# cvlab-epfl/gecco

Hardware: AMD Instinct MI355X
Metric: denoiser_fwd_points_per_sec (higher is better)
Workload: dtype f16/fp6/fp8 mixed (the mixed mode with the point MLP of every layer as ONE launch: fp16 main products + fp6 block-scaled second terms for AdaGN(x) and both weights, the 768-wide hidden layer kept in registers as fp16; the other sites as in the mixed mode; fp32 accumulate, residual stream and statist; 1 GPU; C2 unconditional denoiser forward: B=64/GPU, N=2048, d=384, L=6, I=64, H=8, EDMPrecond(LinearLift(SetTransformer)), mixed fp16 / fp6- and fp8-cross-term MFMA, one-launch point MLP, random-init weights; parallelism=single GPU

## Files before the change

gecco_amd/_lib.py:

```python
from __future__ import annotations

import ctypes as C
import os

_HERE = os.path.dirname(os.path.abspath(__file__))
LIB_PATH = os.environ.get("GECCO_HIP_LIB") or os.path.join(_HERE, "libgecco_hip.so")
ABI_VERSION = 14

c_f = C.c_void_p


class GeccoAdaGN(C.Structure):
    _fields_ = [("scale_w", c_f), ("scale_b", c_f), ("bias_w", c_f), ("bias_b", c_f)]


class GeccoMLP(C.Structure):
    _fields_ = [("w0", c_f), ("b0", c_f), ("alpha", c_f), ("w2", c_f), ("b2", c_f)]


class GeccoLayer(C.Structure):
    _fields_ = [("broadcast_norm", GeccoAdaGN), ("inducers", c_f), ("kv_proj_w", c_f), ("pool_out_w", c_f),
                ("norm_1", GeccoAdaGN), ("bmlp", GeccoMLP), ("norm_2", GeccoAdaGN), ("in_proj_w", c_f),
                ("in_proj_b", c_f), ("unpool_out_w", c_f), ("unpool_out_b", c_f), ("mlp_norm", GeccoAdaGN),
                ("mlp", GeccoMLP)]
# ... 64 lines not shown
    "gecco_split_f16_image_bytes": (sz, [i, i]),
    "gecco_linear_image_ok_f16": (i, [i, i, i, i]),
    "gecco_linear_actbwd_ok": (i, [i, i, i, i]),
    "gecco_linear_actbwd_tiles": (sz, [i, i, i]),
    "gecco_linear_actbwd_f32": (i, [vp, vp, vp, vp, i, vp, vp, vp, i, i, i, i, i, vp, vp]),
    "gecco_linear_act_keep_f32": (i, [vp, vp, vp, vp, i, vp, vp, i, i, i, i, i, vp, vp]),
    "gecco_linear_act_keep_pro_f32": (i, [vp, vp, vp, vp, vp, vp, i, vp, vp, i, i, i, i, i, vp, vp]),
    "gecco_linear_f16io": (i, [vp] * 7 + [i, i, i, i, i, i, i, vp, vp]),
    "gecco_linear_pair_f16io": (i, [vp, vp, vp, i, vp, vp, vp, i, vp, i, i, i, vp, vp]),
    "gecco_mlp_fused_f16": (i, [vp, vp, vp, vp, vp, vp, vp, vp, i, vp, i, i, i, i, vp, vp]),
    "gecco_unpool_outproj_f16": (i, [vp, vp, vp, vp, vp, vp, i, i, i, i, vp, vp]),
    "gecco_unpool_outproj_h8": (i, [vp, vp, vp, vp, vp, vp, i, i, i, i, vp, vp]),
    "gecco_mlp_fused_w": (i, [vp, vp, vp, vp, vp, vp, vp, vp, vp, i, vp, i, i, i, i, vp, vp, vp]),
    "gecco_mlp_fused_w_wsplit_bytes": (sz, [i, i]),
    "gecco_unpool_outproj_h8_wsplit_bytes": (sz, [i, i, i]),
    "gecco_unpool_attn_h8img": (i, [vp, vp, vp, i, i, i, i, vp]),
    "gecco_gemm_tn_x3_f32": (i, [vp, vp, vp, i, i, i, i, i, vp]),
    "gecco_gemm_tn_x3_bias_f32": (i, [vp, vp, vp, vp, i, i, i, i, i, vp]),
    "gecco_gemm_tn_x3_pro_f32": (i, [vp, vp, vp, vp, vp, vp, i, i, i, i, i, vp]),
    "gecco_gemm_tn_f16_f32": (i, [vp, vp, vp, vp, vp, vp, i, i, i, i, i, vp]),
    "gecco_gemm_tn_f16_tiles": (i, [i, i]),
    "gecco_gemm_tn_f16_b16_f32": (i, [vp, vp, vp, vp, i, i, i, i, i, vp]),
    "gecco_gemm_tn_f16_a16_f32": (i, [vp, vp, vp, vp, vp, vp, i, i, i, i, i, vp]),
    "gecco_gemm_tn_f16_ex_f32": (i, [vp, i, vp, i, vp, vp, vp, vp, vp, vp, vp, i, i, i, i, i, vp]),
    "gecco_linear_dotstats_a16_f32": (i, [vp] * 6 + [i, i, i, i, vp, vp]),
    "gecco_linear_astat16_actbwd_h16": (i, [vp] * 4 + [i, vp, vp, i, i, i, i, vp, vp]),
    "gecco_linear_dotstats_f32": (i, [vp] * 5 + [i, i, i, i, i, vp, vp]),
    "gecco_h8_image_bytes": (sz, [i, i]),
    "gecco_linear_h8_train_ok": (i, [i, i, i]),
    "gecco_h8_images_f32": (i, [C.POINTER(GeccoSplitJob), i, vp]),
    "gecco_linear_h8_train_f32": (i, [vp] * 5 + [i, vp, vp, vp, i, vp, vp, i, vp, i, i, i, vp, vp]),
    "gecco_astat16_image_bytes": (sz, [i, i]),
    "gecco_linear_astat16_ok": (i, [i, i, i]),
    "gecco_astat16_images_f32": (i, [C.POINTER(GeccoSplitJob), i, vp]),
    "gecco_linear_astat16_f32": (i, [vp] * 5 + [i, vp, vp, vp, i, vp, vp, i, i, i, i, vp, vp]),
    "gecco_linear_astat16_keep": (i, [vp] * 6 + [i, vp, vp, i, i, i, i, vp, vp]),
    "gecco_linear_astat16_keep_y16": (i, [vp] * 6 + [i, vp, vp, vp, i, i, i, i, vp, vp]),
    "gecco_linear_astat16_actbwd": (i, [vp] * 4 + [i, vp, vp, i, i, i, i, vp, vp]),
    "gecco_linear_act_keep_h16": (i, [vp] * 6 + [i, vp, vp, i, i, i, i, vp, vp]),
    "gecco_set_option": (i, [C.c_char_p, i]),
    "gecco_option_index": (i, [C.c_char_p]),
    "gecco_cast_f16": (i, [c_f, C.c_void_p, C.c_size_t, C.c_void_p]),
    "gecco_linear_astat_f16": (i, [vp, vp, vp, vp, vp, i, vp, vp, vp, i, vp, vp, i, i, i, i, i, vp, vp]),
    "gecco_linear_kvq_f16": (i, [vp, vp, vp, vp, vp, i, vp, vp, vp, i, vp, i, i, i, i, i, i, vp, vp]),
    "gecco_linear_kvq_y16_f16": (i, [vp, vp, vp, vp, vp, i, vp, vp, vp, i, vp, vp, i, i, i, i, i, i, vp, vp]),
    "gecco_linear_h8_img_f32": (i, [vp, vp, vp, vp, vp, vp, i, vp, i, i, i, i, i, vp, vp]),
    "gecco_linear_h8_areg_f32": (i, [vp, vp, vp, vp, vp, vp, i, i, i, i, vp, vp]),
    "gecco_affine_cast_f16": (i, [vp, vp, vp, vp, i, i, i, vp]),
    "gecco_pool_attn_f16in": (i, [vp, vp, vp, i, i, i, i, i, i, vp, sz, vp]),
    "gecco_unpool_attn_f16io": (i, [vp, vp, vp, i, i, i, i, i, i, vp]),
    "gecco_lift0_fold_f32": (i, [vp] * 8 + [i, i, i, vp]),
    "gecco_lift0_rows": (i, [vp, vp, vp, vp, i, i, i, i, i, i, i, vp]),
    "gecco_lift0_pool_f32": (i, [vp] * 5 + [i, i, i, i, vp, sz, vp]),
    "gecco_col_stats_f32": (i, [vp, vp, i, i, i, vp]),
    "gecco_stats_row_tiles": (i, [i]),
    "gecco_adagn_coeffs_f32": (i, [vp, i, i, vp, i, C.POINTER(GeccoAdaGN), vp, vp, i, i, i, fl, vp]),
    "gecco_affine_apply_f32": (i, [vp, vp, vp, vp, i, i, i, vp]),
    "gecco_adagn_f32": (i, [vp, vp, i, C.POINTER(GeccoAdaGN), vp, i, i, i, i, fl, vp, sz, vp]),
    "gecco_adagn_workspace_bytes": (sz, [i, i, i]),
    "gecco_pool_attn_f32": (i, [vp, vp, vp, i, i, i, i, i, vp, sz, vp]),
    "gecco_pool_attn_ex_f32": (i, [vp, vp, vp, i, i, i, i, i, i, vp, sz, vp]),
    "gecco_pool_attn_workspace_bytes": (sz, [i, i, i, i, i]),
    "gecco_unpool_attn_f32": (i, [vp, vp, vp, i, i, i, i, i, vp]),
    "gecco_unpool_attn_ex_f32": (i, [vp, vp, vp, i, i, i, i, i, i, vp]),
    "gecco_pool_attn_lse_f32": (i, [vp, sz, vp, i, i, i, i, i, vp]),
    "gecco_pool_attn_bwd_partials": (i, [i, i, i]),
    "gecco_pool_attn_bwd_f32": (i, [vp] * 7 + [i, i, i, i, i, vp]),
    "gecco_unpool_attn_bwd_partials": (i, [i, i, i]),
    "gecco_unpool_attn_bwd_f32": (i, [vp] * 5 + [i, i, i, i, i, vp]),
    "gecco_pool_attn_bwd_ex_f32": (i, [vp] * 7 + [i, i, i, i, i, i, vp]),
    "gecco_unpool_attn_bwd_ex_f32": (i, [vp] * 5 + [i, i, i, i, i, i, vp]),
    "gecco_edm_coeffs_f32": (i, [vp, fl, vp, i, vp]),
    "gecco_lift_f32": (i, [vp, vp, vp, vp, vp, vp, i, i, i, vp]),
    "gecco_lower_edm_f32": (i, [vp] * 9 + [i, i, i, fl, vp]),
    "gecco_set_transformer_fwd_f32": (i, [C.POINTER(GeccoSetTransformer), vp, vp, vp, i, PP, PP, vp, i, i, vp, sz, vp]),
    "gecco_set_transformer_workspace_bytes": (sz, [C.POINTER(GeccoSetTransformer), i, i]),
    "gecco_linear_lift_fwd_f32": (i, [C.POINTER(GeccoLinearLift), vp, vp, vp, vp, PP, PP, i, i, vp, sz, vp]),
    "gecco_linear_lift_workspace_bytes": (sz, [C.POINTER(GeccoLinearLift), i, i]),
    "gecco_lift_g_f32": (i, [vp, vp, vp, vp, vp, vp, i, i, i, i, vp]),
    "gecco_lower_edm_g_f32": (i, [vp] * 7 + [i, i, i, i, i, fl, vp]),
    "gecco_linear_lift_g_fwd_f32": (i, [C.POINTER(GeccoLinearLiftG), vp, vp, vp, vp, PP, PP, i, i, vp, sz, vp]),
    "gecco_linear_lift_g_workspace_bytes": (sz, [C.POINTER(GeccoLinearLiftG), i, i]),
    "gecco_nchw_to_nhwc_f32": (i, [vp, vp, i, i, i, i, vp]),
    "gecco_bilinear_taps_f32": (i, [vp, i, i, vp, vp, vp, vp, sz, vp]),
    "gecco_ray_lookup_taps_f32": (i, [vp, vp, vp, vp, vp, vp, vp, vp, vp, vp, i, i, vp]),
    "gecco_ray_lookup_f32": (i, [vp, vp, vp, C.POINTER(GeccoReparam), C.POINTER(GeccoPyramid), vp, vp, i, i, vp]),
    "gecco_lookup_row_tiles": (i, [i]),
    "gecco_ray_lookup_bwd_f32": (i, [vp, vp, vp, C.POINTER(GeccoReparam), C.POINTER(GeccoPyramid), vp, PP, i, i, vp]),
    "gecco_ray_lookup_dgeom_f32": (i, [vp, vp, C.POINTER(GeccoReparam), C.POINTER(GeccoPyramid), vp, vp, vp, i, i, vp]),
    "gecco_ray_lookup_bwd_sorted_workspace_bytes": (C.c_size_t, [C.POINTER(GeccoPyramid), i, i]),
    "gecco_ray_lookup_bwd_sorted_f32": (i, [vp, vp, vp, C.POINTER(GeccoReparam), C.POINTER(GeccoPyramid), vp, PP, i, i, vp,
                                            C.c_size_t, vp]),
    "gecco_ray_network_fwd_f32": (i, [C.POINTER(GeccoRayNetwork), vp, vp, vp, C.POINTER(GeccoPyramid), vp, vp, PP, PP,
                                      i, i, vp, sz, vp]),
    "gecco_ray_network_workspace_bytes": (sz, [C.POINTER(GeccoRayNetwork), C.POINTER(GeccoPyramid), i, i]),
    "gecco_gaussian_reparam": (i, [vp, vp, vp, vp, sz, i, i, i, vp]),
    "gecco_uvl_reparam": (i, [vp, vp, vp, vp, db, vp, i, i, i, i, vp]),
    "gecco_gaussian_act_f32": (i, [vp, vp, vp, sz, i, vp]),
    "gecco_relu_f32": (i, [vp, vp, sz, vp]),
    "gecco_relu_bwd_f32": (i, [vp, vp, vp, sz, vp]),
    "gecco_sampler_add_noise_f64": (i, [vp, vp, sz, vp, vp, i, i, vp, vp, vp, sz, i, vp]),
    "gecco_sampler_add_noise_f32": (i, [vp, vp, sz, vp, vp, i, vp, vp, sz, i, vp]),
    "gecco_sampler_euler_f64": (i, [vp, vp, vp, vp, vp, vp, vp, vp, sz, i, vp]),
    "gecco_sampler_heun_f64": (i, [vp, vp, vp, vp, vp, vp, vp, sz, vp]),
    "gecco_sampler_advance": (i, [vp, i, vp]),
    "gecco_sampler_scale_f64": (i, [vp, db, vp, sz, vp]),
# ... 101 lines not shown
```

gecco_amd/csrc/api_model_ops.hip:

```cpp
#include "api_common.h"

#include <math.h>

using namespace gecco_api;

int gecco_api::make_lookup_args(const GeccoReparam* rp, const GeccoPyramid* pyr, LookupArgs* a) {
    if (!pyr || pyr->n_levels < 1 || pyr->n_levels > 4) return fail(-8, "lookup: 1..4 pyramid levels required");
    a->n_levels = pyr->n_levels;
    a->c_total = 0;
    for (int l = 0; l < 4; ++l) {
        const bool on = l < pyr->n_levels;
        a->C[l] = on ? pyr->C[l] : 0;
        a->H[l] = on ? pyr->H[l] : 1;
        a->W[l] = on ? pyr->W[l] : 1;
        a->feat[l] = on ? pyr->feat[l] : nullptr;
        if (on && !pyr->feat[l]) return fail(-1, "lookup: null pyramid level %d", l);
        a->c_total += a->C[l];
    }
    a->texel_f16 = pyr->texel_f16 ? 1 : 0;
    a->out_f16 = 0;
    a->reparam_kind = rp ? rp->kind : 0;
    a->rp_mean = rp ? rp->mean : nullptr;
    a->rp_std = rp ? rp->std : nullptr;
    a->logit_scale = rp ? rp->logit_scale : 1.1f;
    if (a->reparam_kind && (!a->rp_mean || !a->rp_std)) return fail(-1, "lookup: reparam buffers missing");
    return 0;
}

extern "C" {

int gecco_affine_cast_f16(const float* x, const float* a, const float* o, void* y16, int B, int rows, int C,
                          void* stream) {
    if (C % 8) return fail(-2, "affine_cast_f16: C must be a multiple of 8");
    TRY(affine_cast_f16_launch(x, a, o, y16, B, rows, C, (hipStream_t)stream), "affine_cast_f16");
    return 0;
}

int gecco_pool_attn_f16in(const void* KV16, const float* inducers, float* merged, int B, int N, int C, int H, int I,
                          int head_major, void* ws, size_t ws_bytes, void* stream) {
    if (ws_bytes < gecco_pool_attn_workspace_bytes(B, N, C, H, I)) return fail(-7, "pool_attn: workspace too small");
    Carver c(ws);
    const int ns = pool_attn_nsplit(B, N, H);
    float* po = c.f32((size_t)B * H * ns * 64 * (C / H));
    float* pml = c.f32((size_t)B * H * ns * 64 * 2);
    int rc = pool_attn_launch(static_cast<const float*>(KV16), inducers, po, pml, merged, B, N, C, H, I, ns,
                              (hipStream_t)stream, 2, 1, head_major != 0);
    if (rc == -9) return fail(-2, "pool_attn_f16in: head dim must be 16, 32, 48 or 64");
    TRY(rc, "pool_attn_f16in");
    return 0;
}

int gecco_lift0_fold_f32(const float* kv_w, const float* q_w, const float* q_b, const float* lift_w, const float* lift_b, const float* a1,
                         const float* o1, float* mc, int B, int C, int H, void* stream) {
    if (!kv_w || !q_w || !lift_w || !a1 || !o1 || !mc) return fail(-1, "lift0_fold: null argument");
    if (!lift0_supported(C, H)) return fail(-2, "lift0_fold: feature_dim must be a multiple of 8 and of the head count, at most 1024");
    TRY(lift0_fold_launch(kv_w, q_w, q_b, lift_w, lift_b, a1, o1, mc, 0, 3 * C, B, C, (hipStream_t)stream), "lift0_fold");
    return 0;
}

int gecco_lift0_rows(const float* x, const float* coef, const float* mc, void* out, int col0, int ncols, int head_dim, int out_f16,
                     int B, int N, int C, void* stream) {
    if (!x || !coef || !mc || !out) return fail(-1, "lift0_rows: null argument");
    if (ncols <= 0 || ncols % 8 || col0 < 0 || col0 + ncols > 3 * C) return fail(-2, "lift0_rows: columns must be a multiple of 8 inside 0 .. 3 * feature_dim");
    if (head_dim && (!lift0_head_major_ok(head_dim) || ncols % head_dim)) return fail(-2, "lift0_rows: head dim %d has no head-major form", head_dim);
    const Lift0Seg seg{out, col0, ncols, head_dim};
    TRY(lift0_rows_launch(x, coef, mc, &seg, 1, out_f16 != 0, B, N, C, (hipStream_t)stream), "lift0_rows");
    return 0;
}

int gecco_lift0_pool_f32(const float* x, const float* coef, const float* mc, const float* inducers, float* merged, int B, int N, int C,
                         int H, void* ws, size_t ws_bytes, void* stream) {
    if (!x || !coef || !mc || !inducers || !merged || !ws) return fail(-1, "lift0_pool: null argument");
    if (!lift0_pool_supported(C, H)) return fail(-2, "lift0_pool: feature_dim must be a multiple of 8, at most 1024, the head dim a multiple of 4");
    if (ws_bytes < gecco_pool_attn_workspace_bytes(B, N, C, H, 64)) return fail(-7, "lift0_pool: workspace too small");
    Carver c(ws);
    const int ns = pool_attn_nsplit(B, N, H);
    float* po = c.f32((size_t)B * H * ns * 64 * (C / H));
    float* pml = c.f32((size_t)B * H * ns * 64 * 2);
    TRY(lift0_pool_launch(x, coef, mc, inducers, po, pml, B, N, C, H, ns, (hipStream_t)stream), "lift0_pool");
    TRY(pool_merge_launch(po, pml, merged, B, C, H, ns, (hipStream_t)stream), "lift0_pool merge");
    return 0;
}

int gecco_unpool_attn_f16io(const void* q16, const float* kvh, void* out16, int B, int N, int C, int H, int I,
                            int head_major, void* stream) {
    int rc = unpool_attn_launch(static_cast<const float*>(q16), kvh, static_cast<float*>(out16), B, N, C, H, I,
                                (hipStream_t)stream, 2, 1, head_major != 0);
    if (rc == -9) return fail(-2, "unpool_attn_f16io: head dim must be 16, 32, 48 or 64");
    TRY(rc, "unpool_attn_f16io");
    return 0;
}

int gecco_col_stats_f32(const float* x, float* stats, int B, int rows, int C, void* stream) {
    TRY(col_stats_launch(x, stats, B, rows, C, (hipStream_t)stream), "col_stats");
    return 0;
}

int gecco_adagn_coeffs_f32(const float* stats, int T, int rows, const float* t, int ctx_dim, const GeccoAdaGN* p,
                           float* a, float* o, int B, int C, int G, float eps, void* stream) {
    TRY(adagn_coeffs_launch(stats, T, rows, t, ctx_dim, p ? p->scale_w : nullptr, p ? p->scale_b : nullptr,
                            p ? p->bias_w : nullptr, p ? p->bias_b : nullptr, a, o, B, C, G, eps,
                            (hipStream_t)stream), "adagn_coeffs");
    return 0;
}

int gecco_affine_apply_f32(const float* x, const float* a, const float* o, float* y, int B, int rows, int C,
                           void* stream) {
    TRY(affine_apply_launch(x, a, o, y, B, rows, C, (hipStream_t)stream), "affine_apply");
    return 0;
}

size_t gecco_adagn_workspace_bytes(int B, int rows, int C) {
    Carver c(nullptr);
    c.f32((size_t)B * row_tiles_stats(rows) * 2 * C);
    c.f32((size_t)B * C);
    c.f32((size_t)B * C);
    return (c.off + 255) & ~size_t(255);
}

int gecco_adagn_f32(const float* x, const float* t, int ctx_dim, const GeccoAdaGN* p, float* y, int B, int rows,
                    int C, int G, float eps, void* ws, size_t ws_bytes, void* stream) {
    if (ws_bytes < gecco_adagn_workspace_bytes(B, rows, C)) return fail(-7, "adagn: workspace too small");
    Carver c(ws);
    float* stats = c.f32((size_t)B * row_tiles_stats(rows) * 2 * C);
    float* a = c.f32((size_t)B * C);
    float* o = c.f32((size_t)B * C);
    hipStream_t s = (hipStream_t)stream;
    TRY(col_stats_launch(x, stats, B, rows, C, s), "col_stats");
    TRY(adagn_coeffs_launch(stats, row_tiles_stats(rows), rows, t, ctx_dim, p ? p->scale_w : nullptr,
                            p ? p->scale_b : nullptr, p ? p->bias_w : nullptr, p ? p->bias_b : nullptr, a, o, B, C, G,
                            eps, s), "adagn_coeffs");
    TRY(affine_apply_launch(x, a, o, y, B, rows, C, s), "affine_apply");
    return 0;
}
// ... 525 lines not shown
```

gecco_amd/csrc/lift0.hip:

```cpp
#include "common.h"
#include "kernels.h"

namespace {

constexpr float LOG2E = 1.4426950408889634f;
constexpr int FOLD_MAX_C = 1024;
constexpr int ROWS_THREADS = 192;
constexpr int ROWS_TILE = 256;
constexpr int POOL_WAVES = 16;

typedef unsigned u32x4 __attribute__((ext_vector_type(4)));

__global__ __launch_bounds__(256) void lift0_fold_kernel(const float* __restrict__ kv_w, const float* __restrict__ q_w,
                                                         const float* __restrict__ q_b, const float* __restrict__ lift_w,
                                                         const float* __restrict__ lift_b, const float* __restrict__ a1,
                                                         const float* __restrict__ o1, float4* __restrict__ mc, int row0,
                                                         int row1, int C) {
    __shared__ float4 g[FOLD_MAX_C];
    const int b = blockIdx.y;
    for (int k = threadIdx.x; k < C; k += 256) {
        const float a = a1[(size_t)b * C + k], o = o1[(size_t)b * C + k];
        g[k] = make_float4(a * lift_w[k * 3 + 0], a * lift_w[k * 3 + 1], a * lift_w[k * 3 + 2], fmaf(a, lift_b ? lift_b[k] : 0.f, o));
    }
    __syncthreads();
    const int j = row0 + blockIdx.x * 256 + threadIdx.x;
    if (j >= row1) return;
    const f32x4* wr = reinterpret_cast<const f32x4*>(j < 2 * C ? kv_w + (size_t)j * C : q_w + (size_t)(j - 2 * C) * C);
    float4 acc[4];
#pragma unroll
    for (int e = 0; e < 4; ++e) acc[e] = make_float4(0.f, 0.f, 0.f, 0.f);
#pragma unroll 4
    for (int k4 = 0; k4 < C / 4; ++k4) {
        const f32x4 wv = wr[k4];
#pragma unroll
        for (int e = 0; e < 4; ++e) {
            const float4 gk = g[k4 * 4 + e];
            acc[e].x = fmaf(wv[e], gk.x, acc[e].x); acc[e].y = fmaf(wv[e], gk.y, acc[e].y);
            acc[e].z = fmaf(wv[e], gk.z, acc[e].z); acc[e].w = fmaf(wv[e], gk.w, acc[e].w);
        }
    }
    const float bias = (j >= 2 * C && q_b) ? q_b[j - 2 * C] : 0.f;
    mc[(size_t)b * 3 * C + j] = make_float4(((acc[0].x + acc[1].x) + acc[2].x) + acc[3].x, ((acc[0].y + acc[1].y) + acc[2].y) + acc[3].y,
                                            ((acc[0].z + acc[1].z) + acc[2].z) + acc[3].z, (((acc[0].w + acc[1].w) + acc[2].w) + acc[3].w) + bias);
}

struct RowsSeg {
    void* out;
    int col0, gw, ngroups, hm;
    int ld;
};

template <bool F16>
__global__ __launch_bounds__(ROWS_THREADS) void lift0_rows_kernel(const float* __restrict__ x, const float* __restrict__ coef,
                                                                  const float4* __restrict__ mc, RowsSeg s0, RowsSeg s1, int N,
                                                                  int C) {
    __shared__ float xs[ROWS_TILE * 3];
    const int b = blockIdx.z, n0 = blockIdx.x * ROWS_TILE, rows = min(ROWS_TILE, N - n0);
    const bool first = (int)blockIdx.y < s0.ngroups;
    const RowsSeg& s = first ? s0 : s1;
    const int grp = first ? blockIdx.y : blockIdx.y - s0.ngroups;
    const float cin = coef[4 * b + 2];
    for (int i = threadIdx.x; i < rows * 3; i += ROWS_THREADS) xs[i] = cin * x[((size_t)b * N + n0) * 3 + i];
    const int P = s.gw >> 3, piece = threadIdx.x % P, rstep = ROWS_THREADS / P;
    float4 m[8];
    const float4* mp = mc + (size_t)b * 3 * C + s.col0 + grp * s.gw + piece * 8;
#pragma unroll
    for (int e = 0; e < 8; ++e) m[e] = mp[e];
    __syncthreads();
    const size_t base = s.hm ? ((size_t)(b * s.ngroups + grp) * N + n0) * s.gw + piece * 8
                             : ((size_t)b * N + n0) * s.ld + grp * s.gw + piece * 8;
    const size_t rstride = s.hm ? s.gw : s.ld;
    for (int r = threadIdx.x / P; r < rows; r += rstep) {
        const float p0 = xs[r * 3 + 0], p1 = xs[r * 3 + 1], p2 = xs[r * 3 + 2];
        float v[8];
#pragma unroll
        for (int e = 0; e < 8; ++e) v[e] = fmaf(p2, m[e].z, fmaf(p1, m[e].y, fmaf(p0, m[e].x, m[e].w)));
        if (F16) {
            u32x4 o;
#pragma unroll
            for (int e = 0; e < 4; ++e) {
                typedef _Float16 h2 __attribute__((ext_vector_type(2)));
                const h2 pk = {(_Float16)v[2 * e], (_Float16)v[2 * e + 1]};
                o[e] = __builtin_bit_cast(unsigned, pk);
            }
            *reinterpret_cast<u32x4*>(static_cast<_Float16*>(s.out) + base + r * rstride) = o;
        } else {
            float* dst = static_cast<float*>(s.out) + base + r * rstride;
            *reinterpret_cast<f32x4*>(dst) = f32x4{v[0], v[1], v[2], v[3]};
            *reinterpret_cast<f32x4*>(dst + 4) = f32x4{v[4], v[5], v[6], v[7]};
        }
    }
}

__global__ __launch_bounds__(POOL_WAVES * 64) void lift0_pool_kernel(const float* __restrict__ x, const float* __restrict__ coef,
                                                                     const float4* __restrict__ mc, const float* __restrict__ ind,
                                                                     float* __restrict__ part_o, float* __restrict__ part_ml, int N,
                                                                     int C, int H, int HD, int nsplit) {
    constexpr int NW = POOL_WAVES;
    __shared__ float4 red[NW][64];
    __shared__ float redl[NW][64];
    const int lane = threadIdx.x & 63;
    int wave = __builtin_amdgcn_readfirstlane(threadIdx.x >> 6);
    asm volatile("" : "+s"(wave));
    const int bh = blockIdx.x / nsplit, split = blockIdx.x % nsplit;
    const int b = bh / H, hh = bh % H;
    const int ks = (((N + nsplit - 1) / nsplit) + 31) / 32 * 32;
    const int k_begin = split * ks, k_end = min(N, k_begin + ks);
    const int cnt = max(k_end - k_begin, 0);
    const float cin = coef[4 * b + 2];
    const float4* mk = mc + (size_t)b * 3 * C + hh * HD;
    const float4* mv = mk + C;
    typedef const __attribute__((address_space(4))) float* cfloat_p;
    const cfloat_p xp = (cfloat_p)(x + ((size_t)b * N + k_begin) * 3);

    {
        const float scale = LOG2E * rsqrtf((float)HD);
        const float* qi = ind + ((size_t)hh * 64 + lane) * HD;
        float4 acc = make_float4(0.f, 0.f, 0.f, 0.f);
        for (int d0 = wave * 4; d0 < HD; d0 += NW * 4) {
            const f32x4 q4 = *reinterpret_cast<const f32x4*>(qi + d0);
#pragma unroll
            for (int e = 0; e < 4; ++e) {
                const float4 k4 = mk[d0 + e];
                const float qs = q4[e] * scale;
                acc.x = fmaf(qs, k4.x, acc.x); acc.y = fmaf(qs, k4.y, acc.y); acc.z = fmaf(qs, k4.z, acc.z); acc.w = fmaf(qs, k4.w, acc.w);
            }
        }
        red[wave][lane] = acc;
    }
    __syncthreads();
    float4 u = red[0][lane];
#pragma unroll
    for (int w = 1; w < NW; ++w) { const float4 t = red[w][lane]; u.x += t.x; u.y += t.y; u.z += t.z; u.w += t.w; }
    __syncthreads();
    u.x *= cin; u.y *= cin; u.z *= cin;
    auto score = [&](float p0, float p1, float p2) { return fmaf(u.z, p2, fmaf(u.y, p1, fmaf(u.x, p0, u.w))); };

    float m = -INFINITY, l = 0.f, sx = 0.f, sy = 0.f, sz = 0.f;
    for (int k = wave; k < cnt; k += 4 * NW) {
        float p[4][3], sc[4];
#pragma unroll
        for (int j = 0; j < 4; ++j) {
            const int kk = k + j * NW, kc = min(kk, cnt - 1);
#pragma unroll
            for (int e = 0; e < 3; ++e) p[j][e] = xp[kc * 3 + e];
            sc[j] = kk < cnt ? score(p[j][0], p[j][1], p[j][2]) : -INFINITY;
        }
        const float mn = fmaxf(fmaxf(m, fmaxf(sc[0], sc[1])), fmaxf(sc[2], sc[3]));
        const float a = __builtin_amdgcn_exp2f(m - mn);
        l *= a; sx *= a; sy *= a; sz *= a;
#pragma unroll
        for (int j = 0; j < 4; ++j) {
            const float e = __builtin_amdgcn_exp2f(sc[j] - mn);
            l += e;
            sx = fmaf(e, p[j][0], sx); sy = fmaf(e, p[j][1], sy); sz = fmaf(e, p[j][2], sz);
        }
        m = mn;
    }
    redl[wave][lane] = m;
    red[wave][lane] = make_float4(sx, sy, sz, l);
    __syncthreads();
    float M = redl[0][lane];
#pragma unroll
    for (int w = 1; w < NW; ++w) M = fmaxf(M, redl[w][lane]);
    float4 S = make_float4(0.f, 0.f, 0.f, 0.f);
#pragma unroll
    for (int w = 0; w < NW; ++w) {
        const float mw = redl[w][lane];
        const float f = mw == -INFINITY ? 0.f : exp2f(mw - M);
        const float4 t = red[w][lane];
        S.x = fmaf(f, t.x, S.x); S.y = fmaf(f, t.y, S.y); S.z = fmaf(f, t.z, S.z); S.w = fmaf(f, t.w, S.w);
    }
    S.x *= cin; S.y *= cin; S.z *= cin;
    const size_t pbase = ((size_t)bh * nsplit + split) * 64 + lane;
    for (int d = wave; d < HD; d += NW) {
        const float4 v4 = mv[d];
        part_o[pbase * HD + d] = fmaf(v4.z, S.z, fmaf(v4.y, S.y, fmaf(v4.x, S.x, v4.w * S.w)));
    }
    if (wave == 0) {
        part_ml[pbase * 2 + 0] = M;
        part_ml[pbase * 2 + 1] = S.w;
    }
}

int group_width(int ncols) {
    for (int gw : {64, 48, 32, 16, 8})
        if (ncols % gw == 0) return gw;
    return 0;
}

}

bool lift0_supported(int C, int H) { return C >= 8 && C % 8 == 0 && C <= FOLD_MAX_C && H > 0 && C % H == 0; }
bool lift0_head_major_ok(int hd) { return hd >= 8 && hd % 8 == 0 && ROWS_THREADS % (hd / 8) == 0; }
bool lift0_pool_supported(int C, int H) { return lift0_supported(C, H) && (C / H) % 4 == 0; }

int lift0_fold_launch(const float* kv_w, const float* q_w, const float* q_b, const float* lift_w, const float* lift_b, const float* a1,
                      const float* o1, float* mc, int row0, int row1, int B, int C, hipStream_t st) {
    if (C > FOLD_MAX_C || row0 < 0 || row1 > 3 * C || row0 >= row1 || (row0 < 2 * C && !kv_w) || (row1 > 2 * C && !q_w)) return -3;
    if (B <= 0) return 0;
    hipLaunchKernelGGL(lift0_fold_kernel, dim3((row1 - row0 + 255) / 256, B), dim3(256), 0, st, kv_w, q_w, q_b, lift_w, lift_b, a1, o1,
                       reinterpret_cast<float4*>(mc), row0, row1, C);
    return (int)hipGetLastError();
}

int lift0_rows_launch(const float* x, const float* coef, const float* mc, const Lift0Seg* segs, int nseg, int f16, int B, int N, int C,
                      hipStream_t st) {
    if (nseg < 1 || nseg > 2 || B > 65535) return -3;
    if (B <= 0 || N <= 0) return 0;
    RowsSeg rs[2] = {};
    for (int i = 0; i < nseg; ++i) {
        const Lift0Seg& s = segs[i];
        if (s.ncols <= 0 || s.ncols % 8 || s.col0 < 0 || s.col0 + s.ncols > 3 * C) return -3;
        if (s.hd && (!lift0_head_major_ok(s.hd) || s.ncols % s.hd)) return -3;
        const int gw = s.hd ? s.hd : group_width(s.ncols);
        rs[i] = RowsSeg{s.out, s.col0, gw, s.ncols / gw, s.hd != 0, s.ncols};
    }
    const dim3 grid((N + ROWS_TILE - 1) / ROWS_TILE, rs[0].ngroups + rs[1].ngroups, B);
    if (f16) hipLaunchKernelGGL(lift0_rows_kernel<true>, grid, dim3(ROWS_THREADS), 0, st, x, coef, reinterpret_cast<const float4*>(mc), rs[0], rs[1], N, C);
    else hipLaunchKernelGGL(lift0_rows_kernel<false>, grid, dim3(ROWS_THREADS), 0, st, x, coef, reinterpret_cast<const float4*>(mc), rs[0], rs[1], N, C);
    return (int)hipGetLastError();
}

int lift0_pool_launch(const float* x, const float* coef, const float* mc, const float* inducers, float* part_o, float* part_ml, int B,
                      int N, int C, int H, int nsplit, hipStream_t st) {
    if (!lift0_pool_supported(C, H) || nsplit < 1) return -3;
    if (B <= 0) return 0;
    hipLaunchKernelGGL(lift0_pool_kernel, dim3(B * H * nsplit), dim3(POOL_WAVES * 64), 0, st, x, coef, reinterpret_cast<const float4*>(mc), inducers,
                       part_o, part_ml, N, C, H, C / H, nsplit);
    return (int)hipGetLastError();
}
```

gecco_amd/hip_ops.py:

```python
from __future__ import annotations

import contextlib
import ctypes as C
import itertools
import os
import threading
from typing import Mapping, Sequence

import torch
from torch import Tensor

from . import _lib
from ._lib import GeccoAdaGN, GeccoLayer, GeccoLinearLift, GeccoMLP, GeccoSetTransformer, check

GN_EPS = 1e-5

PRECISIONS = {"fp32": 0, "bf16x3": 1, "fp16": 2, "mixed": 3, "w2": 4}
_default_precision = os.environ.get("GECCO_PRECISION", "fp32")


def set_default_precision(name: str) -> None:
    global _default_precision
    if name not in PRECISIONS:
        raise ValueError(f"precision must be one of {sorted(PRECISIONS)}")
# ... 360 lines not shown
    B, _, N, hd = q16.shape
    Cc = H * hd
    out = torch.empty(B, N // 128, Cc // 64, 24576, device=q16.device, dtype=torch.uint8)
    check(lib.gecco_unpool_attn_h8img(_ptr16(q16), _ptr(kvh), C.c_void_p(out.data_ptr()), B, N, Cc, H, _stream()), "gecco_unpool_attn_h8img")
    return out


def affine_cast_f16(x: Tensor, a: Tensor, o: Tensor, out: Tensor | None = None) -> Tensor:
    lib = _lib.load()
    B, rows, Cc = x.shape
    out = torch.empty(B, rows, Cc, device=x.device, dtype=torch.float16) if out is None else out
    check(lib.gecco_affine_cast_f16(_ptr(x), _ptr(a), _ptr(o), _ptr16(out), B, rows, Cc, _stream()), "gecco_affine_cast_f16")
    return out


def pool_attn_f16in(KV16: Tensor, inducers: Tensor, H: int, head_major: bool = False) -> Tensor:
    lib = _lib.load()
    if head_major:
        B, _, N, hd = KV16.shape
        Cc = H * hd
    else:
        B, N, C2 = KV16.shape
        Cc = C2 // 2
    I = inducers.shape[-2]
    merged = torch.empty(B, I, Cc, device=KV16.device, dtype=torch.float32)
    nb = lib.gecco_pool_attn_workspace_bytes(B, N, Cc, H, I)
    ws = _ws(nb, KV16.device)
    check(lib.gecco_pool_attn_f16in(_ptr16(KV16), _ptr(inducers), _ptr(merged), B, N, Cc, H, I, int(head_major),
                                    C.c_void_p(ws.data_ptr()), nb, _stream()), "gecco_pool_attn_f16in")
    return merged


def lift0_fold(kv_w: Tensor, in_proj_w: Tensor, in_proj_b: Tensor | None, lift_w: Tensor, lift_b: Tensor | None, a1: Tensor, o1: Tensor,
               H: int) -> Tensor:
    lib = _lib.load()
    B, Cc = a1.shape
    mc = torch.empty(B, 3 * Cc, 4, device=a1.device, dtype=torch.float32)
    check(lib.gecco_lift0_fold_f32(_ptr(kv_w), _ptr(in_proj_w), _ptr(in_proj_b), _ptr(lift_w), _ptr(lift_b), _ptr(a1), _ptr(o1), _ptr(mc),
                                   B, Cc, H, _stream()), "gecco_lift0_fold_f32")
    return mc


def lift0_rows(x: Tensor, coef: Tensor, mc: Tensor, col0: int, ncols: int, head_dim: int = 0, f16: bool = True) -> Tensor:
    lib = _lib.load()
    B, N, _ = x.shape
    Cc = mc.shape[1] // 3
    shape = (B, ncols // head_dim, N, head_dim) if head_dim else (B, N, ncols)
    out = torch.empty(*shape, device=x.device, dtype=torch.float16 if f16 else torch.float32)
    check(lib.gecco_lift0_rows(_ptr(x), _ptr(coef), _ptr(mc), C.c_void_p(out.data_ptr()), col0, ncols, head_dim, int(f16), B, N, Cc,
                               _stream()), "gecco_lift0_rows")
    return out


def lift0_pool(x: Tensor, coef: Tensor, mc: Tensor, inducers: Tensor, H: int) -> Tensor:
    lib = _lib.load()
    B, N, _ = x.shape
    Cc = mc.shape[1] // 3
    merged = torch.empty(B, 64, Cc, device=x.device, dtype=torch.float32)
    nb = lib.gecco_pool_attn_workspace_bytes(B, N, Cc, H, 64)
    ws = _ws(nb, x.device)
    check(lib.gecco_lift0_pool_f32(_ptr(x), _ptr(coef), _ptr(mc), _ptr(inducers), _ptr(merged), B, N, Cc, H, C.c_void_p(ws.data_ptr()), nb,
                                   _stream()), "gecco_lift0_pool_f32")
    return merged


def unpool_attn_f16io(q16: Tensor, kvh: Tensor, H: int, out: Tensor | None = None, head_major: bool = False) -> Tensor:
    lib = _lib.load()
    if head_major:
        B, _, N, hd = q16.shape
        Cc = H * hd
    else:
        B, N, Cc = q16.shape
    out = torch.empty(B, N, Cc, device=q16.device, dtype=torch.float16) if out is None else out
    check(lib.gecco_unpool_attn_f16io(_ptr16(q16), _ptr(kvh), _ptr16(out), B, N, Cc, H, kvh.shape[1], int(head_major),
                                      _stream()), "gecco_unpool_attn_f16io")
    return out


def linear_pair(A: Tensor, W1: Tensor, b1: Tensor | None, W2: Tensor, b2: Tensor | None,
                pro: tuple[Tensor, Tensor] | None = None, out: tuple[Tensor, Tensor] | None = None,
                precision: str = "fp32", w_image: Tensor | None = None) -> tuple[Tensor, Tensor]:
    lib = _lib.load()
    B, rows, K = A.shape
    n1, n2 = W1.shape[0], W2.shape[0]
    c1, c2 = out if out is not None else (torch.empty(B, rows, n1, device=A.device, dtype=torch.float32),
                                          torch.empty(B, rows, n2, device=A.device, dtype=torch.float32))
    if w_image is not None:
        assert precision in ("bf16x3", "fp16")
        wsplit, W1, W2 = w_image, None, None
    else:
        wsplit = _ws(((n1 + 127) // 128 + (n2 + 127) // 128) * 128 * K * 4, A.device) if precision != "fp32" else None
    check(lib.gecco_linear_pair_f32(_ptr(A), _ptr(W1), _ptr(b1), n1, _ptr(c1), _ptr(W2), _ptr(b2), n2, _ptr(c2),
                                    _ptr(pro[0]) if pro else None, _ptr(pro[1]) if pro else None, B, rows, K,
                                    PRECISIONS[precision], C.c_void_p(wsplit.data_ptr()) if wsplit is not None else None,
                                    _stream()), "gecco_linear_pair_f32")
    return c1, c2


def pool_attn(KV: Tensor, inducers: Tensor, H: int, precision: str = "fp32") -> Tensor:
    lib = _lib.load()
    pr = PRECISIONS[precision]
    B, N, C2 = KV.shape
    Cc = C2 // 2
    I = inducers.shape[-2]
    merged = torch.empty(B, I, Cc, device=KV.device, dtype=torch.float32)
    nb = lib.gecco_pool_attn_workspace_bytes(B, N, Cc, H, I)
    ws = _ws(nb, KV.device)
    check(lib.gecco_pool_attn_ex_f32(_ptr(KV), _ptr(inducers), _ptr(merged), B, N, Cc, H, I, pr,
                                     C.c_void_p(ws.data_ptr()), nb, _stream()), "gecco_pool_attn_ex_f32")
    return merged

# ... 555 lines not shown
```

include/gecco_hip.h:

```cpp
#ifndef GECCO_HIP_H
#define GECCO_HIP_H
#include <stddef.h>
#include <stdint.h>
#ifdef __cplusplus
extern "C" {
#endif

#define GECCO_ABI_VERSION 14

int gecco_abi_version(void);
const char* gecco_build_arch(void);
const char* gecco_last_error(void);

typedef struct GeccoAdaGN {
    const float* scale_w;
    const float* scale_b;
    const float* bias_w;
    const float* bias_b;
} GeccoAdaGN;

typedef struct GeccoMLP {
    const float* w0;
    const float* b0;
    const float* alpha;
// ... 99 lines not shown

int gecco_linear_f16io(const void* A, const float* W, const float* bias, const float* alpha, const float* residual,
                       void* C, float* stats, int B, int rows, int K, int Nout, int act, int a_f16, int c_f16,
                       void* wsplit, void* stream);
int gecco_linear_pair_f16io(const void* A, const float* W1, const float* bias1, int Nout1, void* C1, const float* W2,
                            const float* bias2, int Nout2, void* C2, int B, int rows, int K, void* wsplit,
                            void* stream);
int gecco_linear_astat_f16(const float* x, const float* pro_a, const float* pro_o, const float* W1, const float* bias1,
                           int Nout1, void* C1, const float* W2, const float* bias2, int Nout2, void* C2,
                           const float* alpha, int act, int B, int rows, int K, int head_dim, void* wsplit,
                           void* stream);
int gecco_linear_kvq_f16(const float* x, const float* pro_a, const float* pro_o, const float* W1, const float* bias1, int Nout1,
                         void* C1, const float* W2, const float* bias2, int Nout2, void* C2, int B, int rows, int K, int head_dim,
                         int lo_begin, int lo_end, void* wsplit, void* stream);
int gecco_linear_kvq_y16_f16(const float* x, const float* pro_a, const float* pro_o, const float* W1, const float* bias1, int Nout1,
                             void* C1, const float* W2, const float* bias2, int Nout2, void* C2, void* y16, int B, int rows, int K,
                             int head_dim, int lo_begin, int lo_end, void* wsplit, void* stream);
int gecco_linear_h8_img_f32(const float* x, const float* pro_a, const float* pro_o, const float* W, const float* bias,
                            const float* alpha, int act, void* c_img, int image_kind, int B, int rows, int K, int Nout,
                            void* wsplit, void* stream);
int gecco_linear_h8_areg_f32(const void* a_img, const float* W, const float* bias, const float* residual, float* C, float* stats,
                             int B, int rows, int K, int Nout, void* wsplit, void* stream);
int gecco_mlp_fused_f16(float* x, const float* pro_a, const float* pro_o, const float* W0, const float* b0, const float* W2,
                        const float* b2, const float* alpha, int act, float* stats, int B, int rows, int C, int width,
                        void* wsplit, void* stream);
int gecco_unpool_outproj_f16(float* x, const void* q16, const float* kvh, const float* W, const float* bias, float* stats,
                             int B, int rows, int C, int H, void* wsplit, void* stream);
int gecco_mlp_fused_w(const float* x, float* out, const float* pro_a, const float* pro_o, const float* W0, const float* b0, const float* W2,
                      const float* b2, const float* alpha, int act, float* stats, int B, int rows, int C, int width, void* wsplit, float* dbg_u,
                      void* stream);
size_t gecco_mlp_fused_w_wsplit_bytes(int C, int width);
int gecco_unpool_outproj_h8(float* x, const void* q16, const float* kvh, const float* W, const float* bias, float* stats,
                            int B, int rows, int C, int H, void* wsplit, void* stream);
size_t gecco_unpool_outproj_h8_wsplit_bytes(int B, int C, int H);
int gecco_unpool_attn_h8img(const void* q16, const float* kvh, void* out_img, int B, int N, int C, int H, void* stream);
int gecco_affine_cast_f16(const float* x, const float* a, const float* o, void* y16, int B, int rows, int C,
                          void* stream);
int gecco_pool_attn_f16in(const void* KV16, const float* inducers, float* merged, int B, int N, int C, int H, int I,
                          int head_major, void* ws, size_t ws_bytes, void* stream);
int gecco_unpool_attn_f16io(const void* q16, const float* kvh, void* out16, int B, int N, int C, int H, int I,
                            int head_major, void* stream);

int gecco_pool_attn_f32(const float* KV, const float* inducers, float* merged, int B, int N, int C, int H, int I,
                        void* ws, size_t ws_bytes, void* stream);
int gecco_pool_attn_ex_f32(const float* KV, const float* inducers, float* merged, int B, int N, int C, int H, int I,
                           int precision, void* ws, size_t ws_bytes, void* stream);
size_t gecco_pool_attn_workspace_bytes(int B, int N, int C, int H, int I);
int gecco_lift0_fold_f32(const float* kv_w, const float* q_w, const float* q_b, const float* lift_w, const float* lift_b, const float* a1,
                         const float* o1, float* mc, int B, int C, int H, void* stream);
int gecco_lift0_rows(const float* x, const float* coef, const float* mc, void* out, int col0, int ncols, int head_dim, int out_f16,
                     int B, int N, int C, void* stream);
int gecco_lift0_pool_f32(const float* x, const float* coef, const float* mc, const float* inducers, float* merged, int B, int N, int C,
                         int H, void* ws, size_t ws_bytes, void* stream);

int gecco_pool_attn_lse_f32(const void* ws, size_t ws_bytes, float* lse, int B, int N, int C, int H, int I, void* stream);
int gecco_pool_attn_bwd_partials(int B, int N, int H);
int gecco_pool_attn_bwd_f32(const float* KV, const float* inducers, const float* merged, const float* lse, const float* dO,
                            float* dKV, float* dQ_partials, int B, int N, int C, int H, int I, void* stream);
int gecco_unpool_attn_bwd_partials(int B, int N, int H);
int gecco_unpool_attn_bwd_f32(const float* q, const float* kvh, const float* dO, float* dq, float* dkv_partials, int B, int N,
                              int C, int H, int I, void* stream);
int gecco_pool_attn_bwd_ex_f32(const float* KV, const float* inducers, const float* merged, const float* lse, const float* dO,
                               float* dKV, float* dQ_partials, int B, int N, int C, int H, int I, int precision, void* stream);
int gecco_unpool_attn_bwd_ex_f32(const float* q, const float* kvh, const float* dO, float* dq, float* dkv_partials, int B, int N,
                                 int C, int H, int I, int precision, void* stream);

int gecco_unpool_attn_f32(const float* q, const float* kvh, float* out, int B, int N, int C, int H, int I,
                          void* stream);
int gecco_unpool_attn_ex_f32(const float* q, const float* kvh, float* out, int B, int N, int C, int H, int I,
                             int precision, void* stream);

int gecco_edm_coeffs_f32(const float* sigma, float sigma_data, float* coef, int B, void* stream);
int gecco_lift_f32(const float* x, const float* coef, const float* W, const float* bias, float* out, float* stats,
                   int B, int N, int C, void* stream);
int gecco_lower_edm_f32(const float* feat, const float* x, const float* coef, const float* W, const float* bias,
                        const float* gn_a, const float* gn_o, float* out, float* raw, int B, int N, int C, float eps,
                        void* stream);


int gecco_set_transformer_fwd_f32(const GeccoSetTransformer* st, float* x, const float* t, const float* stats_x,
                                  int stats_T, const float* const* h_in, float* const* h_out, float* stats_out,
                                  int B, int N, void* ws, size_t ws_bytes, void* stream);
size_t gecco_set_transformer_workspace_bytes(const GeccoSetTransformer* st, int B, int N);

typedef struct GeccoLinearLift {
    GeccoSetTransformer inner;
    const float* lift_w;
    const float* lift_b;
    const float* lower_w;
    const float* lower_b;
    float sigma_data;
} GeccoLinearLift;

int gecco_linear_lift_fwd_f32(const GeccoLinearLift* m, const float* x, const float* sigma, float* denoised,
                              float* raw, const float* const* h_in, float* const* h_out, int B, int N, void* ws,
                              size_t ws_bytes, void* stream);
size_t gecco_linear_lift_workspace_bytes(const GeccoLinearLift* m, int B, int N);

#define GECCO_MAX_GEOMETRY_DIM 16
int gecco_lift_g_f32(const float* x, const float* coef, const float* W, const float* bias, float* out, float* stats,
                     int B, int N, int C, int G, void* stream);
int gecco_lower_edm_g_f32(const float* feat, const float* x, const float* coef, const float* W, const float* bias, float* out,
                          float* raw, int B, int N, int C, int G, int do_norm, float eps, void* stream);

typedef struct GeccoLinearLiftG {
    GeccoLinearLift base;
// ... 268 lines not shown
```

Measured before the change: 30.22 million points/s.

## Tile lift0 fold through LDS and stage pool points in shared memory

```diff
diff --git a/gecco_amd/_lib.py b/gecco_amd/_lib.py
--- a/gecco_amd/_lib.py
+++ b/gecco_amd/_lib.py
@@ -140,6 +140,7 @@
     "gecco_lift0_fold_f32": (i, [vp] * 8 + [i, i, i, vp]),
     "gecco_lift0_rows": (i, [vp, vp, vp, vp, i, i, i, i, i, i, i, vp]),
     "gecco_lift0_pool_f32": (i, [vp] * 5 + [i, i, i, i, vp, sz, vp]),
+    "gecco_lift0_pool_split_f32": (i, [vp] * 5 + [i, i, i, i, i, vp, sz, vp]),
     "gecco_col_stats_f32": (i, [vp, vp, i, i, i, vp]),
     "gecco_stats_row_tiles": (i, [i]),
     "gecco_adagn_coeffs_f32": (i, [vp, i, i, vp, i, C.POINTER(GeccoAdaGN), vp, vp, i, i, i, fl, vp]),
diff --git a/gecco_amd/csrc/api_model_ops.hip b/gecco_amd/csrc/api_model_ops.hip
--- a/gecco_amd/csrc/api_model_ops.hip
+++ b/gecco_amd/csrc/api_model_ops.hip
@@ -68,18 +68,26 @@
     return 0;
 }
 
+int gecco_lift0_pool_split_f32(const float* x, const float* coef, const float* mc, const float* inducers, float* merged, int B, int N,
+                               int C, int H, int nsplit, void* ws, size_t ws_bytes, void* stream) {
+    if (!x || !coef || !mc || !inducers || !merged || !ws) return fail(-1, "lift0_pool: null argument");
+    if (!lift0_pool_supported(C, H)) return fail(-2, "lift0_pool: feature_dim must be a multiple of 8, at most 1024, the head dim a multiple of 4");
+    if (nsplit < 1 || nsplit > 64) return fail(-2, "lift0_pool: nsplit must be 1 .. 64");
+    if (B < 0 || N < 0) return fail(-2, "lift0_pool: negative size");
+    if (ws_bytes < (size_t)B * H * nsplit * 64 * (C / H + 2) * sizeof(float)) return fail(-7, "lift0_pool: workspace too small");
+    Carver c(ws);
+    float* po = c.f32((size_t)B * H * nsplit * 64 * (C / H));
+    float* pml = c.f32((size_t)B * H * nsplit * 64 * 2);
+    TRY(lift0_pool_launch(x, coef, mc, inducers, po, pml, B, N, C, H, nsplit, (hipStream_t)stream), "lift0_pool");
+    TRY(pool_merge_launch(po, pml, merged, B, C, H, nsplit, (hipStream_t)stream), "lift0_pool merge");
+    return 0;
+}
+
 int gecco_lift0_pool_f32(const float* x, const float* coef, const float* mc, const float* inducers, float* merged, int B, int N, int C,
                          int H, void* ws, size_t ws_bytes, void* stream) {
-    if (!x || !coef || !mc || !inducers || !merged || !ws) return fail(-1, "lift0_pool: null argument");
     if (!lift0_pool_supported(C, H)) return fail(-2, "lift0_pool: feature_dim must be a multiple of 8, at most 1024, the head dim a multiple of 4");
     if (ws_bytes < gecco_pool_attn_workspace_bytes(B, N, C, H, 64)) return fail(-7, "lift0_pool: workspace too small");
-    Carver c(ws);
-    const int ns = pool_attn_nsplit(B, N, H);
-    float* po = c.f32((size_t)B * H * ns * 64 * (C / H));
-    float* pml = c.f32((size_t)B * H * ns * 64 * 2);
-    TRY(lift0_pool_launch(x, coef, mc, inducers, po, pml, B, N, C, H, ns, (hipStream_t)stream), "lift0_pool");
-    TRY(pool_merge_launch(po, pml, merged, B, C, H, ns, (hipStream_t)stream), "lift0_pool merge");
-    return 0;
+    return gecco_lift0_pool_split_f32(x, coef, mc, inducers, merged, B, N, C, H, pool_attn_nsplit(B, N, H), ws, ws_bytes, stream);
 }
 
 int gecco_unpool_attn_f16io(const void* q16, const float* kvh, void* out16, int B, int N, int C, int H, int I,
diff --git a/gecco_amd/csrc/lift0.hip b/gecco_amd/csrc/lift0.hip
--- a/gecco_amd/csrc/lift0.hip
+++ b/gecco_amd/csrc/lift0.hip
@@ -5,9 +5,13 @@
 
 constexpr float LOG2E = 1.4426950408889634f;
 constexpr int FOLD_MAX_C = 1024;
+constexpr int FOLD_ROWS = 64;
+constexpr int FOLD_KC = 128;
+constexpr int FOLD_SB = 4;
 constexpr int ROWS_THREADS = 192;
 constexpr int ROWS_TILE = 256;
 constexpr int POOL_WAVES = 16;
+constexpr int POOL_CHUNK = 2048;
 
 typedef unsigned u32x4 __attribute__((ext_vector_type(4)));
 
@@ -15,30 +19,68 @@
                                                          const float* __restrict__ q_b, const float* __restrict__ lift_w,
                                                          const float* __restrict__ lift_b, const float* __restrict__ a1,
                                                          const float* __restrict__ o1, float4* __restrict__ mc, int row0,
-                                                         int row1, int C) {
-    __shared__ float4 g[FOLD_MAX_C];
-    const int b = blockIdx.y;
-    for (int k = threadIdx.x; k < C; k += 256) {
-        const float a = a1[(size_t)b * C + k], o = o1[(size_t)b * C + k];
-        g[k] = make_float4(a * lift_w[k * 3 + 0], a * lift_w[k * 3 + 1], a * lift_w[k * 3 + 2], fmaf(a, lift_b ? lift_b[k] : 0.f, o));
-    }
-    __syncthreads();
-    const int j = row0 + blockIdx.x * 256 + threadIdx.x;
-    if (j >= row1) return;
-    const f32x4* wr = reinterpret_cast<const f32x4*>(j < 2 * C ? kv_w + (size_t)j * C : q_w + (size_t)(j - 2 * C) * C);
+                                                         int row1, int C, int B) {
+    __shared__ float ws[FOLD_ROWS][FOLD_KC + 1];
+    __shared__ float4 g[FOLD_SB][FOLD_KC];
+    const int lane = threadIdx.x & 63, wave = threadIdx.x >> 6;
+    const int b = blockIdx.y * FOLD_SB + wave, j0 = row0 + blockIdx.x * FOLD_ROWS, j = j0 + lane;
+    const bool live = b < B && j < row1;
     float4 acc[4];
 #pragma unroll
     for (int e = 0; e < 4; ++e) acc[e] = make_float4(0.f, 0.f, 0.f, 0.f);
+    constexpr int WP = FOLD_ROWS * (FOLD_KC / 4) / 256, GP = FOLD_KC / 64;
+    f32x4 wv[WP];
+    float4 gv[GP];
+    auto fetch = [&](int kc) {
+        const int nk = min(FOLD_KC, C - kc);
+#pragma unroll
+        for (int t = 0; t < GP; ++t) {
+            const int kk = kc + lane + 64 * t;
+            if (b < B && lane + 64 * t < nk) {
+                const float a = a1[(size_t)b * C + kk], o = o1[(size_t)b * C + kk];
+                gv[t] = make_float4(a * lift_w[kk * 3 + 0], a * lift_w[kk * 3 + 1], a * lift_w[kk * 3 + 2], fmaf(a, lift_b ? lift_b[kk] : 0.f, o));
+            }
+        }
+#pragma unroll
+        for (int t = 0; t < WP; ++t) {
+            const int i = threadIdx.x + 256 * t, r = i / (FOLD_KC / 4), c = (i % (FOLD_KC / 4)) * 4, jr = j0 + r;
+            if (jr < row1 && c < nk) {
+                const float* wr = jr < 2 * C ? kv_w + (size_t)jr * C : q_w + (size_t)(jr - 2 * C) * C;
+                wv[t] = *reinterpret_cast<const f32x4*>(wr + kc + c);
+            }
+        }
+    };
+    auto put = [&]() {
+#pragma unroll
+        for (int t = 0; t < GP; ++t) g[wave][lane + 64 * t] = gv[t];
+#pragma unroll
+        for (int t = 0; t < WP; ++t) {
+            const int i = threadIdx.x + 256 * t, r = i / (FOLD_KC / 4), c = (i % (FOLD_KC / 4)) * 4;
+#pragma unroll
+            for (int e = 0; e < 4; ++e) ws[r][c + e] = wv[t][e];
+        }
+    };
+    fetch(0);
+    for (int kc = 0; kc < C; kc += FOLD_KC) {
+        const int nk = min(FOLD_KC, C - kc);
+        if (kc) __syncthreads();
+        put();
+        __syncthreads();
+        if (kc + FOLD_KC < C) fetch(kc + FOLD_KC);
+        if (live) {
 #pragma unroll 4
-    for (int k4 = 0; k4 < C / 4; ++k4) {
-        const f32x4 wv = wr[k4];
-#pragma unroll
-        for (int e = 0; e < 4; ++e) {
-            const float4 gk = g[k4 * 4 + e];
-            acc[e].x = fmaf(wv[e], gk.x, acc[e].x); acc[e].y = fmaf(wv[e], gk.y, acc[e].y);
-            acc[e].z = fmaf(wv[e], gk.z, acc[e].z); acc[e].w = fmaf(wv[e], gk.w, acc[e].w);
-        }
-    }
+            for (int k4 = 0; k4 < nk / 4; ++k4) {
+#pragma unroll
+                for (int e = 0; e < 4; ++e) {
+                    const float w = ws[lane][k4 * 4 + e];
+                    const float4 gk = g[wave][k4 * 4 + e];
+                    acc[e].x = fmaf(w, gk.x, acc[e].x); acc[e].y = fmaf(w, gk.y, acc[e].y);
+                    acc[e].z = fmaf(w, gk.z, acc[e].z); acc[e].w = fmaf(w, gk.w, acc[e].w);
+                }
+            }
+        }
+    }
+    if (!live) return;
     const float bias = (j >= 2 * C && q_b) ? q_b[j - 2 * C] : 0.f;
     mc[(size_t)b * 3 * C + j] = make_float4(((acc[0].x + acc[1].x) + acc[2].x) + acc[3].x, ((acc[0].y + acc[1].y) + acc[2].y) + acc[3].y,
                                             ((acc[0].z + acc[1].z) + acc[2].z) + acc[3].z, (((acc[0].w + acc[1].w) + acc[2].w) + acc[3].w) + bias);
@@ -92,13 +134,14 @@
     }
 }
 
-__global__ __launch_bounds__(POOL_WAVES * 64) void lift0_pool_kernel(const float* __restrict__ x, const float* __restrict__ coef,
-                                                                     const float4* __restrict__ mc, const float* __restrict__ ind,
-                                                                     float* __restrict__ part_o, float* __restrict__ part_ml, int N,
-                                                                     int C, int H, int HD, int nsplit) {
+__global__ __launch_bounds__(POOL_WAVES * 64, 8) void lift0_pool_kernel(const float* __restrict__ x, const float* __restrict__ coef,
+                                                                        const float4* __restrict__ mc, const float* __restrict__ ind,
+                                                                        float* __restrict__ part_o, float* __restrict__ part_ml, int N,
+                                                                        int C, int H, int HD, int nsplit) {
     constexpr int NW = POOL_WAVES;
     __shared__ float4 red[NW][64];
     __shared__ float redl[NW][64];
+    __shared__ __attribute__((aligned(16))) float pts[POOL_CHUNK * 3];
     const int lane = threadIdx.x & 63;
     int wave = __builtin_amdgcn_readfirstlane(threadIdx.x >> 6);
     asm volatile("" : "+s"(wave));
@@ -110,8 +153,22 @@
     const float cin = coef[4 * b + 2];
     const float4* mk = mc + (size_t)b * 3 * C + hh * HD;
     const float4* mv = mk + C;
-    typedef const __attribute__((address_space(4))) float* cfloat_p;
-    const cfloat_p xp = (cfloat_p)(x + ((size_t)b * N + k_begin) * 3);
+    const float* xg = x + ((size_t)b * N + k_begin) * 3;
+
+    constexpr int PP = POOL_CHUNK * 3 / (NW * 64);
+    float pr[PP];
+    auto fetch = [&](int c0, int n) {
+#pragma unroll
+        for (int t = 0; t < PP; ++t) {
+            const int i = threadIdx.x + NW * 64 * t;
+            pr[t] = i < n * 3 ? xg[(size_t)c0 * 3 + i] : 0.f;
+        }
+    };
+    auto put = [&]() {
+#pragma unroll
+        for (int t = 0; t < PP; ++t) pts[threadIdx.x + NW * 64 * t] = pr[t];
+    };
+    fetch(0, min(POOL_CHUNK, cnt));
 
     {
         const float scale = LOG2E * rsqrtf((float)HD);
@@ -128,43 +185,53 @@
         }
         red[wave][lane] = acc;
     }
+    put();
     __syncthreads();
     float4 u = red[0][lane];
-#pragma unroll
+#pragma unroll 4
     for (int w = 1; w < NW; ++w) { const float4 t = red[w][lane]; u.x += t.x; u.y += t.y; u.z += t.z; u.w += t.w; }
     __syncthreads();
     u.x *= cin; u.y *= cin; u.z *= cin;
     auto score = [&](float p0, float p1, float p2) { return fmaf(u.z, p2, fmaf(u.y, p1, fmaf(u.x, p0, u.w))); };
 
     float m = -INFINITY, l = 0.f, sx = 0.f, sy = 0.f, sz = 0.f;
-    for (int k = wave; k < cnt; k += 4 * NW) {
-        float p[4][3], sc[4];
-#pragma unroll
-        for (int j = 0; j < 4; ++j) {
-            const int kk = k + j * NW, kc = min(kk, cnt - 1);
-#pragma unroll
-            for (int e = 0; e < 3; ++e) p[j][e] = xp[kc * 3 + e];
-            sc[j] = kk < cnt ? score(p[j][0], p[j][1], p[j][2]) : -INFINITY;
-        }
-        const float mn = fmaxf(fmaxf(m, fmaxf(sc[0], sc[1])), fmaxf(sc[2], sc[3]));
-        const float a = __builtin_amdgcn_exp2f(m - mn);
-        l *= a; sx *= a; sy *= a; sz *= a;
-#pragma unroll
-        for (int j = 0; j < 4; ++j) {
-            const float e = __builtin_amdgcn_exp2f(sc[j] - mn);
-            l += e;
-            sx = fmaf(e, p[j][0], sx); sy = fmaf(e, p[j][1], sy); sz = fmaf(e, p[j][2], sz);
-        }
-        m = mn;
+    for (int c0 = 0; c0 < cnt; c0 += POOL_CHUNK) {
+        const int n = min(POOL_CHUNK, cnt - c0);
+        if (c0) {
+            __syncthreads();
+            fetch(c0, n);
+            put();
+            __syncthreads();
+        }
+        const int kw = ((n + NW - 1) / NW + 3) & ~3;
+        const int k1 = min(n, (wave + 1) * kw);
+        for (int k = wave * kw; k < k1; k += 4) {
+            const f32x4* pk = reinterpret_cast<const f32x4*>(pts + k * 3);
+            const f32x4 t0 = pk[0], t1 = pk[1], t2 = pk[2];
+            const float p[4][3] = {{t0[0], t0[1], t0[2]}, {t0[3], t1[0], t1[1]}, {t1[2], t1[3], t2[0]}, {t2[1], t2[2], t2[3]}};
+            float sc[4];
+#pragma unroll
+            for (int j = 0; j < 4; ++j) sc[j] = k + j < k1 ? score(p[j][0], p[j][1], p[j][2]) : -INFINITY;
+            const float mn = fmaxf(fmaxf(m, fmaxf(sc[0], sc[1])), fmaxf(sc[2], sc[3]));
+            const float a = __builtin_amdgcn_exp2f(m - mn);
+            l *= a; sx *= a; sy *= a; sz *= a;
+#pragma unroll
+            for (int j = 0; j < 4; ++j) {
+                const float e = __builtin_amdgcn_exp2f(sc[j] - mn);
+                l += e;
+                sx = fmaf(e, p[j][0], sx); sy = fmaf(e, p[j][1], sy); sz = fmaf(e, p[j][2], sz);
+            }
+            m = mn;
+        }
     }
     redl[wave][lane] = m;
     red[wave][lane] = make_float4(sx, sy, sz, l);
     __syncthreads();
     float M = redl[0][lane];
-#pragma unroll
+#pragma unroll 4
     for (int w = 1; w < NW; ++w) M = fmaxf(M, redl[w][lane]);
     float4 S = make_float4(0.f, 0.f, 0.f, 0.f);
-#pragma unroll
+#pragma unroll 4
     for (int w = 0; w < NW; ++w) {
         const float mw = redl[w][lane];
         const float f = mw == -INFINITY ? 0.f : exp2f(mw - M);
@@ -172,14 +239,17 @@
         S.x = fmaf(f, t.x, S.x); S.y = fmaf(f, t.y, S.y); S.z = fmaf(f, t.z, S.z); S.w = fmaf(f, t.w, S.w);
     }
     S.x *= cin; S.y *= cin; S.z *= cin;
-    const size_t pbase = ((size_t)bh * nsplit + split) * 64 + lane;
-    for (int d = wave; d < HD; d += NW) {
-        const float4 v4 = mv[d];
-        part_o[pbase * HD + d] = fmaf(v4.z, S.z, fmaf(v4.y, S.y, fmaf(v4.x, S.x, v4.w * S.w)));
-    }
+    const size_t pbase = ((size_t)bh * nsplit + split) * 64;
     if (wave == 0) {
-        part_ml[pbase * 2 + 0] = M;
-        part_ml[pbase * 2 + 1] = S.w;
+        part_ml[(pbase + lane) * 2 + 0] = M;
+        part_ml[(pbase + lane) * 2 + 1] = S.w;
+    }
+    __syncthreads();
+    if (wave == 0) red[0][lane] = S;
+    __syncthreads();
+    for (int e = threadIdx.x; e < 64 * HD; e += NW * 64) {
+        const float4 v4 = mv[e % HD], Si = red[0][e / HD];
+        part_o[pbase * HD + e] = fmaf(v4.z, Si.z, fmaf(v4.y, Si.y, fmaf(v4.x, Si.x, v4.w * Si.w)));
     }
 }
 
@@ -197,10 +267,10 @@
 
 int lift0_fold_launch(const float* kv_w, const float* q_w, const float* q_b, const float* lift_w, const float* lift_b, const float* a1,
                       const float* o1, float* mc, int row0, int row1, int B, int C, hipStream_t st) {
-    if (C > FOLD_MAX_C || row0 < 0 || row1 > 3 * C || row0 >= row1 || (row0 < 2 * C && !kv_w) || (row1 > 2 * C && !q_w)) return -3;
+    if (C > FOLD_MAX_C || C % 8 || B > 65535 * FOLD_SB || row0 < 0 || row1 > 3 * C || row0 >= row1 || (row0 < 2 * C && !kv_w) || (row1 > 2 * C && !q_w)) return -3;
     if (B <= 0) return 0;
-    hipLaunchKernelGGL(lift0_fold_kernel, dim3((row1 - row0 + 255) / 256, B), dim3(256), 0, st, kv_w, q_w, q_b, lift_w, lift_b, a1, o1,
-                       reinterpret_cast<float4*>(mc), row0, row1, C);
+    hipLaunchKernelGGL(lift0_fold_kernel, dim3((row1 - row0 + FOLD_ROWS - 1) / FOLD_ROWS, (B + FOLD_SB - 1) / FOLD_SB), dim3(256), 0, st, kv_w, q_w,
+                       q_b, lift_w, lift_b, a1, o1, reinterpret_cast<float4*>(mc), row0, row1, C, B);
     return (int)hipGetLastError();
 }
 
diff --git a/gecco_amd/hip_ops.py b/gecco_amd/hip_ops.py
--- a/gecco_amd/hip_ops.py
+++ b/gecco_amd/hip_ops.py
@@ -436,11 +436,17 @@
     return out
 
 
-def lift0_pool(x: Tensor, coef: Tensor, mc: Tensor, inducers: Tensor, H: int) -> Tensor:
+def lift0_pool(x: Tensor, coef: Tensor, mc: Tensor, inducers: Tensor, H: int, nsplit: int = 0) -> Tensor:
     lib = _lib.load()
     B, N, _ = x.shape
     Cc = mc.shape[1] // 3
     merged = torch.empty(B, 64, Cc, device=x.device, dtype=torch.float32)
+    if nsplit:
+        nb = B * H * nsplit * 64 * (Cc // H + 2) * 4
+        ws = _ws(nb, x.device)
+        check(lib.gecco_lift0_pool_split_f32(_ptr(x), _ptr(coef), _ptr(mc), _ptr(inducers), _ptr(merged), B, N, Cc, H, nsplit,
+                                             C.c_void_p(ws.data_ptr()), nb, _stream()), "gecco_lift0_pool_split_f32")
+        return merged
     nb = lib.gecco_pool_attn_workspace_bytes(B, N, Cc, H, 64)
     ws = _ws(nb, x.device)
     check(lib.gecco_lift0_pool_f32(_ptr(x), _ptr(coef), _ptr(mc), _ptr(inducers), _ptr(merged), B, N, Cc, H, C.c_void_p(ws.data_ptr()), nb,
diff --git a/include/gecco_hip.h b/include/gecco_hip.h
--- a/include/gecco_hip.h
+++ b/include/gecco_hip.h
@@ -175,6 +175,8 @@
                      int B, int N, int C, void* stream);
 int gecco_lift0_pool_f32(const float* x, const float* coef, const float* mc, const float* inducers, float* merged, int B, int N, int C,
                          int H, void* ws, size_t ws_bytes, void* stream);
+int gecco_lift0_pool_split_f32(const float* x, const float* coef, const float* mc, const float* inducers, float* merged, int B, int N,
+                               int C, int H, int nsplit, void* ws, size_t ws_bytes, void* stream);
 
 int gecco_pool_attn_lse_f32(const void* ws, size_t ws_bytes, float* lse, int B, int N, int C, int H, int I, void* stream);
 int gecco_pool_attn_bwd_partials(int B, int N, int H);
```

Result: faster. 30.56 million points/s (median of 6 runs) (+1.1%).
